# jgrss/cultionet

Hardware: AMD Instinct MI355X
Metric: train_chips_per_sec (higher is better)
Workload: dtype f32

## Files before the change

### cultionet_amd/csrc/cn_wgrad.hip

```cpp
#include <cstdlib>
#include "cn_common.h"
#include "cn_profile.h"
#include "cn_slicesum.h"

#define WG_MAX_TAPS 9
#define WG_BC 32
#define WG_NS 4
#define WG_NB 13
#define WG_KS 8
#define WG_U 4
#define WG_KB 16

struct CnWgradGeom {
  int N;
  int A, Hs, Ws; long sbs; long scs;
  int Bc, Hb, Wb; long bbs; long bcs;
  double flops;
  int s;
  int T;
  int offy[WG_MAX_TAPS], offx[WG_MAX_TAPS];
  int min_oy, min_ox;
  long sa;
  int PR, Wsp, pitch_s;
  int rows_b, pitch_b, plane_b;
  int a_tiles;
  int chunks_per_img, total_chunks, chunks_per_split;
  int b_lds_off;
  int buf_stride;
  int nbuf;
  int colsplit;
  int G, spg;
  const float* gS[4];
  const float* gB[4];
  float* gdW[4];
  long slice_stride;
  int grid_x, grid_y, grid_z;
  int mq_lo, mq_hi;
};

typedef __attribute__((address_space(3))) void* cn_lds_ptr;
typedef const __attribute__((address_space(1))) void* cn_gbl_ptr;

__device__ float cn_zero_line[64];

__device__ __forceinline__ void cn_glds4(const float* src, float* lds_wave_base) {
  __builtin_amdgcn_global_load_lds((cn_gbl_ptr)src, (cn_lds_ptr)lds_wave_base, 4, 0, 0);
}

template <int T>
__global__ __launch_bounds__(256) void cn_wgrad_kernel(const float* __restrict__ S, const float* __restrict__ Bg,
                                                      float* __restrict__ dW, const CnWgradGeom g) {
  extern __shared__ __attribute__((aligned(16))) float smem[];

  const int tid = threadIdx.x, lane = tid & 63, wid = tid >> 6;
  const int half = lane >> 5, l31 = lane & 31;
  const int at = wid % g.a_tiles, kp = wid / g.a_tiles, kparts = 4 / g.a_tiles;
  int bx, by, bz;
  if (!cn_xcd_block(g.grid_x, g.grid_y, g.grid_x * g.grid_y * g.grid_z, bx, by, bz)) return;
  const int a0 = by * g.a_tiles * 32;
  const int b0 = bx * WG_BC;
  const int npix = g.PR * g.Wsp;
  const float* zero = cn_zero_line + lane;

  int so[WG_NS];
#pragma unroll
  for (int i = 0; i < WG_NS; ++i) {
    const int e = lane + i * 64;
    if (e < npix) {
      const int r = e / g.Wsp, c = e - r * g.Wsp;
      so[i] = (r << 16) | ((c < g.Ws) ? c : 0xFFFF);
    } else {
      so[i] = -2;
    }
  }
  int bo[WG_NB];
#pragma unroll
  for (int i = 0; i < WG_NB; ++i) {
    const int e = lane + i * 64;
    if (e < g.plane_b) {
      const int r = e / g.pitch_b;
      bo[i] = (r << 16) | (e - r * g.pitch_b);
    } else {
      bo[i] = -1;
    }
  }

  int boff[T];
#pragma unroll
  for (int j = 0; j < T; ++j) {
    const int n = j * 32 + l31;
    const int bl = n / T, t = n - bl * T;
    boff[j] = bl * g.plane_b + (g.offy[t] - g.min_oy) * g.pitch_b + (g.offx[t] - g.min_ox) + half * g.s;
  }
  const int aoff = (at * 32 + l31) * g.pitch_s + half;

  f32x16 acc[T];
#pragma unroll
  for (int j = 0; j < T; ++j)
#pragma unroll
    for (int r = 0; r < 16; ++r) acc[j][r] = 0.f;

  const int HWs = g.Hs * g.Ws, HWb = g.Hb * g.Wb;
  const int arows = g.a_tiles * 32;
  int chunk = bz * g.chunks_per_split;
  int chunk_end = chunk + g.chunks_per_split;
  if (chunk_end > g.total_chunks) chunk_end = g.total_chunks;

  const int steps = npix >> 1;
  const int q_begin = (steps * kp) / kparts, q_end = (steps * (kp + 1)) / kparts;
  const int e_begin = q_begin * 2;
  const int r_begin = e_begin / g.Wsp, c_begin = e_begin - r_begin * g.Wsp;

  auto stage = [&](int ck, int buf) {
    float* s_lds = smem + buf * g.buf_stride;
    float* b_lds = s_lds + g.b_lds_off;
    const int n = ck / g.chunks_per_img;
    const int gy0 = (ck - n * g.chunks_per_img) * g.PR;
    const int pr = (g.Hs - gy0 < g.PR) ? g.Hs - gy0 : g.PR;
    const float* Sn = S + (long)n * g.sbs + (long)gy0 * g.Ws;
    for (int a = wid; a < arows; a += 4) {
      const bool aok = (a0 + a) < g.A;
      const float* Sa = Sn + (long)(a0 + a) * g.scs;
#pragma unroll
      for (int i = 0; i < WG_NS; ++i) {
        if (i * 64 < npix) {
          if (so[i] != -2) {
            const int r = so[i] >> 16, c = so[i] & 0xFFFF;
            const float* src = (aok && c != 0xFFFF && r < pr) ? Sa + r * g.Ws + c : zero;
            cn_glds4(src, s_lds + a * g.pitch_s + i * 64);
          }
        }
      }
    }
    const float* Bn = Bg + (long)n * g.bbs;
    const int iy0 = gy0 * g.s + g.min_oy;
    for (int bl = wid; bl < WG_BC; bl += 4) {
      const bool bok = (b0 + bl) < g.Bc;
      const float* Bb = Bn + (long)(b0 + bl) * g.bcs;
#pragma unroll
      for (int i = 0; i < WG_NB; ++i) {
        if (i * 64 < g.plane_b) {
          if (bo[i] >= 0) {
            const int iy = iy0 + (bo[i] >> 16), ix = g.min_ox + (bo[i] & 0xFFFF);
            const float* src = (bok && iy >= 0 && iy < g.Hb && ix >= 0 && ix < g.Wb) ? Bb + iy * g.Wb + ix : zero;
            cn_glds4(src, b_lds + bl * g.plane_b + i * 64);
          }
        }
      }
    }
  };

  int cur = 0;
  if (chunk < chunk_end && g.nbuf == 2) stage(chunk, 0);
  for (; chunk < chunk_end; ++chunk) {
    if (g.nbuf == 1) {
      __syncthreads();
      stage(chunk, 0);
    }
    __syncthreads();
    if (g.nbuf == 2 && chunk + 1 < chunk_end) stage(chunk + 1, cur ^ 1);
    const float* s_lds = smem + cur * g.buf_stride;
    const float* b_lds = s_lds + g.b_lds_off;
    int r = r_begin, c = c_begin;
    for (int q = q_begin; q < q_end; ++q) {
      const float av = s_lds[aoff + r * g.Wsp + c];
      const int bbase = (r * g.s) * g.pitch_b + c * g.s;
#pragma unroll
      for (int j = 0; j < T; ++j) {
        const float bv = b_lds[boff[j] + bbase];
        acc[j] = __builtin_amdgcn_mfma_f32_32x32x2f32(av, bv, acc[j], 0, 0, 0);
      }
      c += 2;
      if (c >= g.Wsp) { c = 0; ++r; }
    }
    if (g.nbuf == 2) cur ^= 1;
  }

#pragma unroll
  for (int j = 0; j < T; ++j) {
    const int n = j * 32 + l31;
    const int bl = n / T;
    const bool bok = (b0 + bl) < g.Bc;
#pragma unroll
    for (int r = 0; r < 16; ++r) {
      const int a = a0 + at * 32 + (r & 3) + 8 * (r >> 2) + 4 * half;
      if (bok && a < g.A) atomicAdd(dW + (long)a * g.sa + (long)b0 * T + n, acc[j][r]);
    }
  }
}

__device__ float cn_zero_line16[256];

#ifdef CNW_STAMP
__device__ unsigned long long cnw_stamps[256];
#define CNW_ST() do { if (do_stamp && stamp_i < 256) cnw_stamps[stamp_i++] = __builtin_amdgcn_s_memtime(); } while (0)
extern "C" int cn_wgrad_read_stamps(unsigned long long* out) {
  return hipMemcpyFromSymbol(out, HIP_SYMBOL(cnw_stamps), sizeof(unsigned long long) * 256) == hipSuccess ? 0 : -2;
}
#else
#define CNW_ST() do { } while (0)
#endif

__device__ __forceinline__ void cn_glds16(const float* src, float* lds_wave_base) {
  __builtin_amdgcn_global_load_lds((cn_gbl_ptr)src, (cn_lds_ptr)lds_wave_base, 16, 0, 0);
}

template <int T, int S_>
__global__ __launch_bounds__(256) void cn_wgrad_vec_kernel(const float* __restrict__ S0, const float* __restrict__ Bg0,
                                                          float* __restrict__ dW0, const CnWgradGeom g) {
  extern __shared__ __attribute__((aligned(16))) float smem[];
  const int tid = threadIdx.x, lane = tid & 63;
  const int wid = __builtin_amdgcn_readfirstlane(tid >> 6);
  const int half = lane >> 5, l31 = lane & 31;
  const int at = wid % g.a_tiles, kp = wid / g.a_tiles, kparts = 4 / g.a_tiles;
  int bx, by, bz;
  if (!cn_xcd_block(g.grid_x, g.grid_y, g.grid_x * g.grid_y * g.grid_z, bx, by, bz)) return;
  const int grp = g.G > 1 ? bz / g.spg : 0;
  const int split = bz - grp * g.spg;
  const float* __restrict__ S = g.G > 1 ? g.gS[grp] : S0;
  const float* __restrict__ Bg = g.G > 1 ? g.gB[grp] : Bg0;
  float* __restrict__ dW = (g.G > 1 && g.slice_stride == 0) ? g.gdW[grp] : dW0;
  const int a0 = by * g.a_tiles * 32;
  const int b0 = bx * WG_BC;
  const int npix = g.PR * g.Ws;
  const int n4s = npix >> 2;
  const int n4b = g.plane_b >> 2;
  const float* zero = cn_zero_line16 + 4 * lane;
  const int HWs = g.Hs * g.Ws, HWb = g.Hb * g.Wb;

  int boff[T], ox[T];
#pragma unroll
  for (int j = 0; j < T; ++j) {
    const int n = j * 32 + l31;
    const int bl = n / T, t = n - bl * T;
    boff[j] = bl * g.plane_b + (g.offy[t] - g.min_oy) * g.Wb + (g.offx[t] - g.min_ox) + half * g.s;
    ox[j] = g.offx[t] + half * g.s;
  }
  const int aoff = (at * 32 + l31) * g.pitch_s + half;

  f32x16 acc[T];
#pragma unroll
  for (int j = 0; j < T; ++j)
#pragma unroll
    for (int r = 0; r < 16; ++r) acc[j][r] = 0.f;

  const int arows = g.a_tiles * 32;
  int chunk = split * g.chunks_per_split;
  int chunk_end = chunk + g.chunks_per_split;
  if (chunk_end > g.total_chunks) chunk_end = g.total_chunks;

  const int steps = npix >> 1;
  const int q_begin = (steps * kp) / kparts, q_end = (steps * (kp + 1)) / kparts;
  const int e_begin = q_begin * 2;
  const int r_begin = e_begin / g.Ws, c_begin = e_begin - r_begin * g.Ws;

  constexpr unsigned WG_IDLE = 0xFFFFFFFFu;
  unsigned so[WG_KS], bo[WG_KB];
  {
    const int nsp = arows * n4s, nbp = WG_BC * n4b;
#pragma unroll
    for (int k = 0; k < WG_KS; ++k) {
      const int p = (wid + 4 * k) * 64 + lane;
      const int a = p / n4s, pc = p - a * n4s;
      so[k] = (p < nsp && (a0 + a) < g.A) ? (unsigned)(((long)(a0 + a) * g.scs + 4 * pc) * 4) : WG_IDLE;
    }
#pragma unroll
    for (int k = 0; k < WG_KB; ++k) {
      const int p = (wid + 4 * k) * 64 + lane;
      const int bl = p / n4b, pi = p - bl * n4b;
      bo[k] = (p < nbp && (b0 + bl) < g.Bc) ? (unsigned)(((long)(b0 + bl) * g.bcs + 4 * pi) * 4) : WG_IDLE;
    }
  }
  auto stage = [&](int ck, int buf) {
    float* s_lds = smem + buf * g.buf_stride;
    float* b_lds = s_lds + g.b_lds_off;
    const int n = ck / g.chunks_per_img;
    const int gy0 = (ck - n * g.chunks_per_img) * g.PR;
    const int nsp = arows * n4s, nbp = WG_BC * n4b;
    {
      const int fs0 = gy0 * g.Ws;
      const char* sbase = reinterpret_cast<const char*>(S + (long)n * g.sbs + fs0);
      if (fs0 + npix <= (int)g.scs) {
#pragma unroll
        for (int k = 0; k < WG_KS; ++k)
          if ((wid + 4 * k) * 64 < nsp && so[k] != WG_IDLE)
            cn_glds16(reinterpret_cast<const float*>(sbase + so[k]), s_lds + (wid + 4 * k) * 256);
      } else {
#pragma unroll
        for (int k = 0; k < WG_KS; ++k) {
          if ((wid + 4 * k) * 64 < nsp && so[k] != WG_IDLE) {
            const int p = (wid + 4 * k) * 64 + lane;
            const int pc = p % n4s;
            const bool ok = (fs0 + 4 * pc + 3) < (int)g.scs;
            const float* src = ok ? reinterpret_cast<const float*>(sbase + so[k]) : zero;
            cn_glds16(src, s_lds + (wid + 4 * k) * 256);
          }
        }
      }
    }
    {
      const int start = (gy0 * g.s + g.min_oy) * g.Wb + g.min_ox;
      const int f0 = (start >> 2) << 2;
      const char* bbase = reinterpret_cast<const char*>(Bg + (long)n * g.bbs + f0);
      if (f0 >= 0 && f0 + g.plane_b <= (int)g.bcs) {
#pragma unroll
        for (int k = 0; k < WG_KB; ++k)
          if ((wid + 4 * k) * 64 < nbp && bo[k] != WG_IDLE)
            cn_glds16(reinterpret_cast<const float*>(bbase + bo[k]), b_lds + (wid + 4 * k) * 256);
      } else {
#pragma unroll
        for (int k = 0; k < WG_KB; ++k) {
          if ((wid + 4 * k) * 64 < nbp && bo[k] != WG_IDLE) {
            const int p = (wid + 4 * k) * 64 + lane;
            const int fq = f0 + 4 * (p % n4b);
            const bool ok = fq >= 0 && (fq + 3) < (int)g.bcs;
            const float* src = ok ? reinterpret_cast<const float*>(bbase + bo[k]) : zero;
            cn_glds16(src, b_lds + (wid + 4 * k) * 256);
          }
        }
      }
    }
  };

  int cur = 0;
#ifdef CNW_STAMP
  const bool do_stamp = T == 9 && S_ == 1 && blockIdx.x == 8 && tid == 0;
  int stamp_i = 0;
#endif
  CNW_ST();
  if (chunk < chunk_end && g.nbuf == 2) stage(chunk, 0);
  for (; chunk < chunk_end; ++chunk) {
    CNW_ST();
    if (g.nbuf == 1) {
      __syncthreads();
      stage(chunk, 0);
    }
    __syncthreads();
    CNW_ST();
    if (g.nbuf == 2 && chunk + 1 < chunk_end) stage(chunk + 1, cur ^ 1);
    CNW_ST();
    const float* s_lds = smem + cur * g.buf_stride;
    const float* b_lds = s_lds + g.b_lds_off;
    const int gy0c = (chunk % g.chunks_per_img) * g.PR;
    const int start = (gy0c * g.s + g.min_oy) * g.Wb + g.min_ox;
    const int sh = start - ((start >> 2) << 2);
    {
      const int nq_row = g.Ws >> 1;
      const int q_lo = (nq_row * kp) / kparts, q_hi = (nq_row * (kp + 1)) / kparts;
      const int seg0 = min(max(g.mq_lo, q_lo), q_hi), seg1 = max(min(g.mq_hi, q_hi), seg0);
      for (int r = 0; r < g.PR; ++r) {
        const float* ap = s_lds + aoff + r * g.Ws;
        const float* bp[T];
#pragma unroll
        for (int j = 0; j < T; ++j) bp[j] = b_lds + boff[j] + sh + (r * S_) * g.Wb;
        int q = q_lo;
        for (; q < seg0; ++q) {
          const float av = ap[2 * q];
          const int cs = 2 * q * S_;
          float bv[T];
#pragma unroll
          for (int j = 0; j < T; ++j) bv[j] = bp[j][cs];
#pragma unroll
          for (int j = 0; j < T; ++j) {
            const float b_ = ((unsigned)(cs + ox[j]) < (unsigned)g.Wb) ? bv[j] : 0.f;
            acc[j] = __builtin_amdgcn_mfma_f32_32x32x2f32(av, b_, acc[j], 0, 0, 0);
          }
        }
        CNW_ST();
        if constexpr (T == 1) {
          for (; q + WG_U <= seg1; q += WG_U) {
            const float* apq = ap + 2 * q;
#pragma unroll
            for (int u = 0; u < WG_U; ++u)
              acc[0] = __builtin_amdgcn_mfma_f32_32x32x2f32(apq[2 * u], (bp[0] + 2 * q * S_)[2 * u * S_], acc[0], 0, 0, 0);
          }
        } else {
          constexpr int GS = 2;
          const int ng = (seg1 - q) / GS;
          if (ng > 0) {
            float a0[GS], a1[GS], b0[GS][T], b1[GS][T];
#define WG_LOADG(qq_, a_, b_)                                                    \
  {                                                                              \
    const float* apq_ = ap + 2 * (qq_);                                          \
    _Pragma("unroll") for (int u = 0; u < GS; ++u) a_[u] = apq_[2 * u];          \
    _Pragma("unroll") for (int j = 0; j < T; ++j) {                              \
      const float* bq_ = bp[j] + 2 * (qq_) * S_;                                 \
      _Pragma("unroll") for (int u = 0; u < GS; ++u) b_[u][j] = bq_[2 * u * S_]; \
    }                                                                            \
  }
#define WG_MFMAG(a_, b_)                                                                                   \
  {                                                                                                        \
    _Pragma("unroll") for (int u = 0; u < GS; ++u)                                                         \
        _Pragma("unroll") for (int j = 0; j < T; ++j)                                                      \
            acc[j] = __builtin_amdgcn_mfma_f32_32x32x2f32(a_[u], b_[u][j], acc[j], 0, 0, 0);               \
  }
            WG_LOADG(q, a0, b0);
            int i = 0;
            for (; i + 2 <= ng; i += 2) {
              WG_LOADG(q + GS * (i + 1), a1, b1);
              WG_MFMAG(a0, b0);
              if (i + 2 < ng) WG_LOADG(q + GS * (i + 2), a0, b0);
              WG_MFMAG(a1, b1);
            }
            if (i < ng) WG_MFMAG(a0, b0);
#undef WG_LOADG
#undef WG_MFMAG
            q += GS * ng;
          }
        }
        CNW_ST();
        for (; q < seg1; ++q) {
          const float av = ap[2 * q];
          float bv[T];
#pragma unroll
          for (int j = 0; j < T; ++j) bv[j] = bp[j][2 * q * S_];
#pragma unroll
          for (int j = 0; j < T; ++j) acc[j] = __builtin_amdgcn_mfma_f32_32x32x2f32(av, bv[j], acc[j], 0, 0, 0);
        }
        for (; q < q_hi; ++q) {
          const float av = ap[2 * q];
          const int cs = 2 * q * S_;
          float bv[T];
#pragma unroll
          for (int j = 0; j < T; ++j) bv[j] = bp[j][cs];
#pragma unroll
          for (int j = 0; j < T; ++j) {
            const float b_ = ((unsigned)(cs + ox[j]) < (unsigned)g.Wb) ? bv[j] : 0.f;
            acc[j] = __builtin_amdgcn_mfma_f32_32x32x2f32(av, b_, acc[j], 0, 0, 0);
          }
        }
      }
    }
    CNW_ST();
    if (g.nbuf == 2) cur ^= 1;
  }
  CNW_ST();

  if (kparts > 1) {
    __syncthreads();
    float* red = smem;
    if (kp > 0) {
      float* rp = red + (long)((kp - 1) * g.a_tiles + at) * (T * 16 * 64) + lane;
#pragma unroll
      for (int j = 0; j < T; ++j)
#pragma unroll
        for (int r = 0; r < 16; ++r) rp[(j * 16 + r) * 64] = acc[j][r];
    }
    __syncthreads();
    if (kp > 0) return;
    for (int k = 1; k < kparts; ++k) {
      const float* rp = red + (long)((k - 1) * g.a_tiles + at) * (T * 16 * 64) + lane;
#pragma unroll
      for (int j = 0; j < T; ++j)
#pragma unroll
        for (int r = 0; r < 16; ++r) acc[j][r] += rp[(j * 16 + r) * 64];
    }
  }
  float* dWs = dW + (long)bz * g.slice_stride;
#pragma unroll
  for (int j = 0; j < T; ++j) {
    const int n = j * 32 + l31;
    const int bl = n / T;
    const bool bok = (b0 + bl) < g.Bc;
#pragma unroll
    for (int r = 0; r < 16; ++r) {
      const int a = a0 + at * 32 + (r & 3) + 8 * (r >> 2) + 4 * half;
      if (bok && a < g.A) {
        if (g.slice_stride != 0) dWs[(long)a * g.sa + (long)b0 * T + n] = acc[j][r];
        else atomicAdd(dW + (long)a * g.sa + (long)b0 * T + n, acc[j][r]);
      }
    }
  }
}

#define WG3_WAVES 12
#define WG3_KS 3
#define WG3_KB 6
template <int S_>
__global__ __launch_bounds__(WG3_WAVES * 64) void cn_wgrad_vec3_kernel(const float* __restrict__ S0,
                                                                       const float* __restrict__ Bg0,
                                                                       float* __restrict__ dW0, const CnWgradGeom g) {
  extern __shared__ __attribute__((aligned(16))) float smem[];
  constexpr int T = 3;
  const int tid = threadIdx.x, lane = tid & 63;
  const int wid = __builtin_amdgcn_readfirstlane(tid >> 6);
  const int half = lane >> 5, l31 = lane & 31;
  const int at = wid % g.a_tiles;
  const int ky = (wid / g.a_tiles) % 3;
  const int kp = wid / (g.a_tiles * 3), kparts = WG3_WAVES / (g.a_tiles * 3);
  int bx, by, bz;
  if (!cn_xcd_block(g.grid_x, g.grid_y, g.grid_x * g.grid_y * g.grid_z, bx, by, bz)) return;
  const int grp = g.G > 1 ? bz / g.spg : 0;
  const int split = bz - grp * g.spg;
  const float* __restrict__ S = g.G > 1 ? g.gS[grp] : S0;
  const float* __restrict__ Bg = g.G > 1 ? g.gB[grp] : Bg0;
  float* __restrict__ dW = (g.G > 1 && g.slice_stride == 0) ? g.gdW[grp] : dW0;
  const int a0 = by * g.a_tiles * 32;
  const int b0 = bx * WG_BC;
  const int npix = g.PR * g.Ws;
  const int n4s = npix >> 2;
  const int n4b = g.plane_b >> 2;
  const float* zero = cn_zero_line16 + 4 * lane;

  int boff[T], ox[T];
#pragma unroll
  for (int j = 0; j < T; ++j) {
    const int n = j * 32 + l31;
    const int bl = n / 3, t = ky * 3 + (n - bl * 3);
    boff[j] = bl * g.plane_b + (g.offy[t] - g.min_oy) * g.Wb + (g.offx[t] - g.min_ox) + half * g.s;
    ox[j] = g.offx[t] + half * g.s;
  }
  const int aoff = (at * 32 + l31) * g.pitch_s + half;

  f32x16 acc[T];
#pragma unroll
  for (int j = 0; j < T; ++j)
#pragma unroll
    for (int r = 0; r < 16; ++r) acc[j][r] = 0.f;

  const int arows = g.a_tiles * 32;
  int chunk = split * g.chunks_per_split;
  int chunk_end = chunk + g.chunks_per_split;
  if (chunk_end > g.total_chunks) chunk_end = g.total_chunks;

  constexpr unsigned WG_IDLE = 0xFFFFFFFFu;
  unsigned so[WG3_KS], bo[WG3_KB];
  {
    const int nsp = arows * n4s, nbp = WG_BC * n4b;
#pragma unroll
    for (int k = 0; k < WG3_KS; ++k) {
      const int p = (wid + WG3_WAVES * k) * 64 + lane;
      const int a = p / n4s, pc = p - a * n4s;
      so[k] = (p < nsp && (a0 + a) < g.A) ? (unsigned)(((long)(a0 + a) * g.scs + 4 * pc) * 4) : WG_IDLE;
    }
#pragma unroll
    for (int k = 0; k < WG3_KB; ++k) {
      const int p = (wid + WG3_WAVES * k) * 64 + lane;
      const int bl = p / n4b, pi = p - bl * n4b;
      bo[k] = (p < nbp && (b0 + bl) < g.Bc) ? (unsigned)(((long)(b0 + bl) * g.bcs + 4 * pi) * 4) : WG_IDLE;
    }
  }
  auto stage = [&](int ck, int buf) {
    float* s_lds = smem + buf * g.buf_stride;
    float* b_lds = s_lds + g.b_lds_off;
    const int n = ck / g.chunks_per_img;
    const int gy0 = (ck - n * g.chunks_per_img) * g.PR;
    const int nsp = arows * n4s, nbp = WG_BC * n4b;
    {
      const int fs0 = gy0 * g.Ws;
      const char* sbase = reinterpret_cast<const char*>(S + (long)n * g.sbs + fs0);
      const bool inside = fs0 + npix <= (int)g.scs;
#pragma unroll
      for (int k = 0; k < WG3_KS; ++k) {
        if ((wid + WG3_WAVES * k) * 64 < nsp && so[k] != WG_IDLE) {
          const float* src = reinterpret_cast<const float*>(sbase + so[k]);
          if (!inside) {
            const int p = (wid + WG3_WAVES * k) * 64 + lane;
            if (!((fs0 + 4 * (p % n4s) + 3) < (int)g.scs)) src = zero;
          }
          cn_glds16(src, s_lds + (wid + WG3_WAVES * k) * 256);
        }
      }
    }
    {
      const int start = (gy0 * g.s + g.min_oy) * g.Wb + g.min_ox;
      const int f0 = (start >> 2) << 2;
      const char* bbase = reinterpret_cast<const char*>(Bg + (long)n * g.bbs + f0);
      const bool inside = f0 >= 0 && f0 + g.plane_b <= (int)g.bcs;
#pragma unroll
      for (int k = 0; k < WG3_KB; ++k) {
        if ((wid + WG3_WAVES * k) * 64 < nbp && bo[k] != WG_IDLE) {
          const float* src = reinterpret_cast<const float*>(bbase + bo[k]);
          if (!inside) {
            const int p = (wid + WG3_WAVES * k) * 64 + lane;
            const int fq = f0 + 4 * (p % n4b);
            if (!(fq >= 0 && (fq + 3) < (int)g.bcs)) src = zero;
          }
          cn_glds16(src, b_lds + (wid + WG3_WAVES * k) * 256);
        }
      }
    }
  };

  int cur = 0;
  if (chunk < chunk_end && g.nbuf == 2) stage(chunk, 0);
  for (; chunk < chunk_end; ++chunk) {
    if (g.nbuf == 1) {
      __syncthreads();
      stage(chunk, 0);
    }
    __syncthreads();
    if (g.nbuf == 2 && chunk + 1 < chunk_end) stage(chunk + 1, cur ^ 1);
    const float* s_lds = smem + cur * g.buf_stride;
    const float* b_lds = s_lds + g.b_lds_off;
    const int gy0c = (chunk % g.chunks_per_img) * g.PR;
    const int start = (gy0c * g.s + g.min_oy) * g.Wb + g.min_ox;
    const int sh = start - ((start >> 2) << 2);
    const int nq_row = g.Ws >> 1;
    const int q_lo = (nq_row * kp) / kparts, q_hi = (nq_row * (kp + 1)) / kparts;
    const int seg0 = min(max(g.mq_lo, q_lo), q_hi), seg1 = max(min(g.mq_hi, q_hi), seg0);
    for (int r = 0; r < g.PR; ++r) {
      const float* ap = s_lds + aoff + r * g.Ws;
      const float* bp[T];
#pragma unroll
      for (int j = 0; j < T; ++j) bp[j] = b_lds + boff[j] + sh + (r * S_) * g.Wb;
      int q = q_lo;
      for (; q < seg0; ++q) {
        const float av = ap[2 * q];
        const int cs = 2 * q * S_;
        float bv[T];
#pragma unroll
        for (int j = 0; j < T; ++j) bv[j] = bp[j][cs];
#pragma unroll
        for (int j = 0; j < T; ++j) {
          const float b_ = ((unsigned)(cs + ox[j]) < (unsigned)g.Wb) ? bv[j] : 0.f;
          acc[j] = __builtin_amdgcn_mfma_f32_32x32x2f32(av, b_, acc[j], 0, 0, 0);
        }
      }
      {
        constexpr int GS = 3;
        const int ng = (seg1 - q) / GS;
        if (ng > 0) {
          float a0[GS], a1[GS], b0[GS][T], b1[GS][T];
#define WG3_LOADG(qq_, a_, b_)                                                   \
  {                                                                              \
    const float* apq_ = ap + 2 * (qq_);                                          \
    _Pragma("unroll") for (int u = 0; u < GS; ++u) a_[u] = apq_[2 * u];          \
    _Pragma("unroll") for (int j = 0; j < T; ++j) {                              \
      const float* bq_ = bp[j] + 2 * (qq_) * S_;                                 \
      _Pragma("unroll") for (int u = 0; u < GS; ++u) b_[u][j] = bq_[2 * u * S_]; \
    }                                                                            \
  }
#define WG3_MFMAG(a_, b_)                                                                                  \
  {                                                                                                        \
    _Pragma("unroll") for (int u = 0; u < GS; ++u)                                                         \
        _Pragma("unroll") for (int j = 0; j < T; ++j)                                                      \
            acc[j] = __builtin_amdgcn_mfma_f32_32x32x2f32(a_[u], b_[u][j], acc[j], 0, 0, 0);               \
  }
          WG3_LOADG(q, a0, b0);
          int i = 0;
          for (; i + 2 <= ng; i += 2) {
            WG3_LOADG(q + GS * (i + 1), a1, b1);
            WG3_MFMAG(a0, b0);
            if (i + 2 < ng) WG3_LOADG(q + GS * (i + 2), a0, b0);
            WG3_MFMAG(a1, b1);
          }
          if (i < ng) WG3_MFMAG(a0, b0);
#undef WG3_LOADG
#undef WG3_MFMAG
          q += GS * ng;
        }
      }
      for (; q < seg1; ++q) {
        const float av = ap[2 * q];
        float bv[T];
#pragma unroll
        for (int j = 0; j < T; ++j) bv[j] = bp[j][2 * q * S_];
#pragma unroll
        for (int j = 0; j < T; ++j) acc[j] = __builtin_amdgcn_mfma_f32_32x32x2f32(av, bv[j], acc[j], 0, 0, 0);
      }
      for (; q < q_hi; ++q) {
        const float av = ap[2 * q];
        const int cs = 2 * q * S_;
        float bv[T];
#pragma unroll
        for (int j = 0; j < T; ++j) bv[j] = bp[j][cs];
#pragma unroll
        for (int j = 0; j < T; ++j) {
          const float b_ = ((unsigned)(cs + ox[j]) < (unsigned)g.Wb) ? bv[j] : 0.f;
          acc[j] = __builtin_amdgcn_mfma_f32_32x32x2f32(av, b_, acc[j], 0, 0, 0);
        }
      }
    }
    if (g.nbuf == 2) cur ^= 1;
  }

  if (kparts > 1) {
    __syncthreads();
    float* red = smem;
    const int slot = ky * g.a_tiles + at;
    if (kp > 0) {
      float* rp = red + (long)((kp - 1) * g.a_tiles * 3 + slot) * (T * 16 * 64) + lane;
#pragma unroll
      for (int j = 0; j < T; ++j)
#pragma unroll
        for (int r = 0; r < 16; ++r) rp[(j * 16 + r) * 64] = acc[j][r];
    }
    __syncthreads();
    if (kp > 0) return;
    for (int k = 1; k < kparts; ++k) {
      const float* rp = red + (long)((k - 1) * g.a_tiles * 3 + slot) * (T * 16 * 64) + lane;
#pragma unroll
      for (int j = 0; j < T; ++j)
#pragma unroll
        for (int r = 0; r < 16; ++r) acc[j][r] += rp[(j * 16 + r) * 64];
    }
  }
  float* dWs = dW + (long)bz * g.slice_stride;
#pragma unroll
  for (int j = 0; j < T; ++j) {
    const int n = j * 32 + l31;
    const int bl = n / 3, t = ky * 3 + (n - bl * 3);
    const bool bok = (b0 + bl) < g.Bc;
#pragma unroll
    for (int r = 0; r < 16; ++r) {
      const int a = a0 + at * 32 + (r & 3) + 8 * (r >> 2) + 4 * half;
      if (bok && a < g.A) {
        float* d = (g.slice_stride != 0 ? dWs : dW) + (long)a * g.sa + (long)(b0 + bl) * 9 + t;
        if (g.slice_stride != 0) *d = acc[j][r];
        else atomicAdd(d, acc[j][r]);
      }
    }
  }
}

struct CnWgradReduceArgs {
  const float* part; long slice_stride; int nslices; long n;
  float* dW[4];
};
__global__ __launch_bounds__(256) void cn_wgrad_reduce_kernel(const CnWgradReduceArgs a) {
  const long i = blockIdx.x * 256L + threadIdx.x;
  if (i >= a.n) return;
  const float* part = a.part + (long)blockIdx.z * a.nslices * a.slice_stride;
  float* dW = a.dW[blockIdx.z];
  float s0 = 0.f, s1 = 0.f;
  int k = blockIdx.y;
  for (; k + (int)gridDim.y < a.nslices; k += 2 * gridDim.y) {
    s0 += part[(long)k * a.slice_stride + i];
    s1 += part[(long)(k + gridDim.y) * a.slice_stride + i];
  }
  if (k < a.nslices) s0 += part[(long)k * a.slice_stride + i];
  if (gridDim.y == 1) dW[i] += s0 + s1;
  else atomicAdd(dW + i, s0 + s1);
}

template <int T>
static int cn_wgrad_launch_vec(const float* S, const float* Bg, float* dW, CnWgradGeom g, float* ws, long ws_floats,
                               hipStream_t stream) {
  if (g.scs % 4 || g.bcs % 4 || g.sbs % 4 || g.bbs % 4 || (g.Ws & 1)) return CN_ERR_ARG;
  g.Wsp = g.Ws;
  g.PR = 128 / g.Ws;
  if (g.PR < 1) g.PR = 1;
  if (g.PR > g.Hs) g.PR = g.Hs;
  while (g.PR > 1 && (g.PR * g.Ws) % 4 != 0) --g.PR;
  if ((g.PR * g.Ws) % 4 != 0 && g.Ws % 2 == 0 && 2 * g.Ws <= 256) g.PR = 2;
  if ((g.PR * g.Ws) % 4 != 0 || g.PR * g.Ws > 256) return CN_ERR_ARG;
  int max_oy = g.min_oy, max_ox = g.min_ox;
  for (int t = 0; t < g.T; ++t) {
    if (g.offy[t] > max_oy) max_oy = g.offy[t];
    if (g.offx[t] > max_ox) max_ox = g.offx[t];
  }
  g.rows_b = (g.PR - 1) * g.s + (max_oy - g.min_oy) + 1;
  g.pitch_b = g.Wb;
  g.plane_b = ((g.rows_b - 1) * g.Wb + (g.Ws - 1) * g.s + (max_ox - g.min_ox) + 4 + 3) / 4 * 4;
  if (WG_BC * g.plane_b > WG_KB * 4 * 256) return CN_ERR_ARG;
  g.pitch_s = g.PR * g.Ws;
  g.a_tiles = g.A > 32 ? 2 : 1;
  size_t lds;
  for (;;) {
    g.b_lds_off = (g.a_tiles * 32 * g.pitch_s + 255) / 256 * 256;
    g.buf_stride = g.b_lds_off + (WG_BC * g.plane_b + 255) / 256 * 256;
    lds = (size_t)g.buf_stride * sizeof(float);
    if ((lds <= 160 * 1024 && g.a_tiles * 32 * g.pitch_s <= WG_KS * 4 * 256) || g.a_tiles == 1) break;
    g.a_tiles >>= 1;
  }
  if (lds > 160 * 1024 || g.a_tiles * 32 * g.pitch_s > WG_KS * 4 * 256) return CN_ERR_ARG;
  g.nbuf = (2 * lds <= 160 * 1024) ? 2 : 1;
  lds *= g.nbuf;
  {
    const size_t red = (size_t)(4 / g.a_tiles - 1) * g.a_tiles * T * 16 * 64 * sizeof(float);
    if (red > lds) lds = red;
  }
  g.chunks_per_img = (g.Hs + g.PR - 1) / g.PR;
  g.total_chunks = g.N * g.chunks_per_img;
  const int gx = (g.Bc + WG_BC - 1) / WG_BC, gy = (g.A + g.a_tiles * 32 - 1) / (g.a_tiles * 32);
  if (g.G < 1) {
    g.G = 1;
    g.gS[0] = S; g.gB[0] = Bg; g.gdW[0] = dW;
  }
  for (int i = 0; i < g.G; ++i)
    if ((reinterpret_cast<uintptr_t>(g.gS[i]) & 15) || (reinterpret_cast<uintptr_t>(g.gB[i]) & 15)) return CN_ERR_ARG;
  const int slots = (lds * 2 <= 160 * 1024) ? 512 : 256;
  int splits = slots / (gx * gy * g.G);
  if (splits > g.total_chunks) splits = g.total_chunks;
  if (splits < 1) splits = 1;
  g.chunks_per_split = (g.total_chunks + splits - 1) / splits;
  splits = (g.total_chunks + g.chunks_per_split - 1) / g.chunks_per_split;
  static bool attr_set = false;
  if (!attr_set) {
    (void)hipFuncSetAttribute((const void*)cn_wgrad_vec_kernel<T, 1>, hipFuncAttributeMaxDynamicSharedMemorySize,
                              160 * 1024);
    (void)hipFuncSetAttribute((const void*)cn_wgrad_vec_kernel<T, 2>, hipFuncAttributeMaxDynamicSharedMemorySize,
                              160 * 1024);
    attr_set = true;
  }
  if (g.s != 1 && g.s != 2) return CN_ERR_ARG;
  {
    const int nq_row = g.Ws / 2;
    int lo = (-g.min_ox + 2 * g.s - 1) / (2 * g.s);
    if (lo < 0) lo = 0;
    int hi_num = g.Wb - max_ox - g.s;
    int hi = hi_num <= 0 ? 0 : (hi_num + 2 * g.s - 1) / (2 * g.s);
    if (lo > nq_row) lo = nq_row;
    if (hi > nq_row) hi = nq_row;
    if (hi < lo) hi = lo;
    g.mq_lo = lo;
    g.mq_hi = hi;
  }
  cn_prof_name("cn_wgrad_vec_kernel<%d, %d>", T, g.s == 1 ? 1 : 2);
  cn_prof_desc("wgrad_vec<%d> G%d N%d A%d %dx%d Bc%d %dx%d s%d grid%dx%dx%d nbuf%d", T, g.G, g.N, g.A, g.Hs, g.Ws, g.Bc,
               g.Hb, g.Wb, g.s, gx, gy, splits, g.nbuf);
  g.spg = splits;
  g.grid_x = gx; g.grid_y = gy; g.grid_z = splits * g.G;
  const dim3 grid(cn_xcd_grid((long)gx * gy * splits * g.G));
  const int kparts = 4 / g.a_tiles;
  const long dw_floats = (long)g.A * g.sa;
  const long nslices = splits;
  float* out = g.gdW[0];
  g.slice_stride = 0;
  if (nslices >= 16 && ws != nullptr && nslices * g.G * dw_floats <= ws_floats) {
    g.slice_stride = dw_floats;
    out = ws;
  }
  if (T == 9) cn_prof_name("cn_wgrad_vec3_kernel<%d>", g.s == 1 ? 1 : 2);
  cn_prof_bytes(4.0 * g.G * ((double)g.N * g.A * g.Hs * g.Ws + (double)g.N * g.Bc * g.Hb * g.Wb + (double)dw_floats));
  cn_prof_before(stream);
  if (T == 9) {
    static bool attr3 = false;
    if (!attr3) {
      (void)hipFuncSetAttribute((const void*)cn_wgrad_vec3_kernel<1>, hipFuncAttributeMaxDynamicSharedMemorySize, 160 * 1024);
      (void)hipFuncSetAttribute((const void*)cn_wgrad_vec3_kernel<2>, hipFuncAttributeMaxDynamicSharedMemorySize, 160 * 1024);
      attr3 = true;
    }
    if (g.s == 1)
      CN_LAUNCH((cn_wgrad_vec3_kernel<1>), grid, dim3(WG3_WAVES * 64), lds, stream, g.gS[0], g.gB[0], out, g);
    else
      CN_LAUNCH((cn_wgrad_vec3_kernel<2>), grid, dim3(WG3_WAVES * 64), lds, stream, g.gS[0], g.gB[0], out, g);
  } else if (g.s == 1)
    CN_LAUNCH((cn_wgrad_vec_kernel<T, 1>), grid, dim3(256), lds, stream, g.gS[0], g.gB[0], out, g);
  else
    CN_LAUNCH((cn_wgrad_vec_kernel<T, 2>), grid, dim3(256), lds, stream, g.gS[0], g.gB[0], out, g);
  cn_prof_after(stream, T == 9 ? 2 : 3, g.flops * g.G);
  if (g.slice_stride != 0) {
    CnSliceSum js[4] = {};
    for (int i = 0; i < g.G; ++i) {
      js[i].part = ws + (long)i * nslices * g.slice_stride; js[i].dw = g.gdW[i]; js[i].slice_stride = g.slice_stride;
      js[i].n = dw_floats; js[i].nslices = (int)nslices; js[i].kind = 0;
    }
    if (cn_ss_push(js, g.G)) return cn_check_launch();
    CnWgradReduceArgs ra = {ws, g.slice_stride, (int)nslices, dw_floats, {g.gdW[0], g.gdW[1], g.gdW[2], g.gdW[3]}};
    CN_LAUNCH(cn_wgrad_reduce_kernel,
                       dim3((unsigned)((dw_floats + 255) / 256), nslices > 128 ? 16 : 1, g.G), dim3(256), 0, stream,
                       ra);
  }
  return cn_check_launch();
}

template <int T>
static int cn_wgrad_launch_t(const float* S, const float* Bg, float* dW, CnWgradGeom g, hipStream_t stream) {
  g.Wsp = (g.Ws + 1) & ~1;
  if (g.Wsp > 64 * WG_NS) return CN_ERR_LDS;
  g.PR = 128 / g.Wsp;
  if (g.PR < 1) g.PR = 1;
  if (g.PR > g.Hs) g.PR = g.Hs;
  int max_oy = g.min_oy, max_ox = g.min_ox;
  for (int t = 0; t < g.T; ++t) {
    if (g.offy[t] > max_oy) max_oy = g.offy[t];
    if (g.offx[t] > max_ox) max_ox = g.offx[t];
  }
  for (;;) {
    g.rows_b = (g.PR - 1) * g.s + (max_oy - g.min_oy) + 1;
    g.pitch_b = (g.Wsp - 1) * g.s + (max_ox - g.min_ox) + 1;
    g.plane_b = g.rows_b * g.pitch_b;
    if (g.plane_b <= 64 * WG_NB || g.PR == 1) break;
    --g.PR;
  }
  if (g.plane_b > 64 * WG_NB) return CN_ERR_LDS;
  g.pitch_s = (g.PR * g.Wsp) | 1;
  g.a_tiles = g.A > 64 ? 4 : (g.A > 32 ? 2 : 1);
  if (g.a_tiles == 4) g.a_tiles = 2;
  size_t lds;
  for (;;) {
    g.b_lds_off = (g.a_tiles * 32 * g.pitch_s + 3) / 4 * 4;
    g.buf_stride = (g.b_lds_off + WG_BC * g.plane_b + 3) / 4 * 4;
    lds = (size_t)g.buf_stride * sizeof(float);
    if (lds <= 160 * 1024 || g.a_tiles == 1) break;
    g.a_tiles >>= 1;
  }
  if (lds > 160 * 1024) return CN_ERR_LDS;
  g.nbuf = (2 * lds <= 160 * 1024) ? 2 : 1;
  lds *= g.nbuf;
  g.chunks_per_img = (g.Hs + g.PR - 1) / g.PR;
  g.total_chunks = g.N * g.chunks_per_img;
  const int gx = (g.Bc + WG_BC - 1) / WG_BC, gy = (g.A + g.a_tiles * 32 - 1) / (g.a_tiles * 32);
  int splits = (768 + gx * gy - 1) / (gx * gy);
  if (splits > g.total_chunks) splits = g.total_chunks;
  if (splits < 1) splits = 1;
  g.chunks_per_split = (g.total_chunks + splits - 1) / splits;
  splits = (g.total_chunks + g.chunks_per_split - 1) / g.chunks_per_split;
  static bool attr_set = false;
  if (!attr_set) {
    (void)hipFuncSetAttribute((const void*)cn_wgrad_kernel<T>, hipFuncAttributeMaxDynamicSharedMemorySize,
                              160 * 1024);
    attr_set = true;
  }
  cn_prof_name("cn_wgrad_kernel<%d>", T);
  cn_prof_desc("wgrad_dw<%d> N%d A%d %dx%d Bc%d %dx%d s%d grid%dx%dx%d", T, g.N, g.A, g.Hs, g.Ws, g.Bc, g.Hb, g.Wb, g.s,
               gx, gy, splits);
  g.grid_x = gx; g.grid_y = gy; g.grid_z = splits;
  cn_prof_before(stream);
  CN_LAUNCH((cn_wgrad_kernel<T>), dim3(cn_xcd_grid((long)gx * gy * splits)), dim3(256), lds, stream, S, Bg,
                     dW, g);
  cn_prof_after(stream, T == 9 ? 2 : 3, g.flops);
  return cn_check_launch();
}

struct CnPadSet {
  const float* src; long sbs; long scs;
  float* dst; int C, H, W, Wp, cs;
};
#define CN_PAD_MAX_SETS 8
struct CnPadArgs {
  CnPadSet set[CN_PAD_MAX_SETS];
  int cbegin[CN_PAD_MAX_SETS + 1];
  int nsets;
};

__global__ __launch_bounds__(256) void cn_pad_planes_kernel(const CnPadArgs a) {
  int si = 0;
#pragma unroll 1
  for (int i = 1; i < a.nsets; ++i)
    if ((int)blockIdx.y >= a.cbegin[i]) si = i;
  const CnPadSet& p = a.set[si];
  const int c = blockIdx.y - a.cbegin[si], b = blockIdx.z;
  const float* sp = p.src + b * p.sbs + (long)c * p.scs;
  float* dp = p.dst + ((long)b * p.C + c) * p.cs;
  for (int i = blockIdx.x * 256 + threadIdx.x; i < p.cs; i += gridDim.x * 256) {
    const int r = i / p.Wp, col = i - r * p.Wp;
    dp[i] = (r < p.H && col < p.W) ? sp[r * p.W + col] : 0.f;
  }
}

static int cn_pad_planes(CnPadArgs& a, int B, hipStream_t stream) {
  if (a.nsets == 0) return CN_OK;
  int cs = 0, ctot = 0;
  for (int i = 0; i < a.nsets; ++i) {
    a.cbegin[i] = ctot;
    ctot += a.set[i].C;
    if (a.set[i].cs > cs) cs = a.set[i].cs;
  }
  a.cbegin[a.nsets] = ctot;
  int bx = (cs + 1023) / 1024;
  if (bx < 1) bx = 1;
  CN_LAUNCH(cn_pad_planes_kernel, dim3(bx, ctot, B), dim3(256), 0, stream, a);
  return cn_check_launch();
}

static int cn_wgrad_generic_g(int G, const float* const* Ss, long sbs, int A, int Hs, int Ws, const float* const* Bgs,
                              long bbs, int Bc, int Hb, int Wb, int s, int KH, int KW, int dil, int pad,
                              float* const* dWs, int N, float* ws, long ws_floats, hipStream_t stream) {
  if (G < 1 || G > 4) return CN_ERR_ARG;
  CnWgradGeom g = {};
  g.N = N; g.A = A; g.Hs = Hs; g.Ws = Ws; g.sbs = sbs; g.Bc = Bc; g.Hb = Hb; g.Wb = Wb; g.bbs = bbs; g.s = s;
  g.scs = (long)Hs * Ws; g.bcs = (long)Hb * Wb;
  g.T = KH * KW;
  if (N <= 0 || A <= 0 || Bc <= 0 || Hs <= 0 || Ws <= 0) return CN_OK;
  g.flops = 2.0 * N * Hs * Ws * (double)A * Bc * g.T;
  for (int ky = 0; ky < KH; ++ky)
    for (int kx = 0; kx < KW; ++kx) {
      g.offy[ky * KW + kx] = ky * dil - pad;
      g.offx[ky * KW + kx] = kx * dil - pad;
    }
  g.min_oy = -pad; g.min_ox = -pad;
  g.sa = (long)Bc * g.T;
  if (g.T != 1 && g.T != 9) return CN_ERR_ARG;
  g.G = G;
  for (int i = 0; i < G; ++i) { g.gS[i] = Ss[i]; g.gB[i] = Bgs[i]; g.gdW[i] = dWs[i]; }
  const bool ws_ok = ws != nullptr && (reinterpret_cast<uintptr_t>(ws) & 15) == 0;
  int rc = g.T == 1 ? cn_wgrad_launch_vec<1>(Ss[0], Bgs[0], dWs[0], g, ws_ok ? ws : nullptr, ws_floats, stream)
                    : cn_wgrad_launch_vec<9>(Ss[0], Bgs[0], dWs[0], g, ws_ok ? ws : nullptr, ws_floats, stream);
  if (rc != CN_ERR_ARG) return rc;
  if (ws_ok) {
    const int Wsp = (Ws + 1) & ~1;
    const long scs = ((long)Hs * Wsp + 3) / 4 * 4, bcs = ((long)Hb * Wb + 3) / 4 * 4;
    const long need_s = (long)N * A * scs, need_b = (long)N * Bc * bcs;
    CnWgradGeom gp = g;
    CnPadArgs pa = {};
    float* w = ws;
    long need = 0;
    bool any_s = false, any_b = false;
    for (int i = 0; i < G; ++i) {
      const bool s_ok = (g.scs % 4 == 0) && (sbs % 4 == 0) && !(Ws & 1) && !(reinterpret_cast<uintptr_t>(Ss[i]) & 15);
      const bool b_ok = (g.bcs % 4 == 0) && (bbs % 4 == 0) && !(reinterpret_cast<uintptr_t>(Bgs[i]) & 15);
      any_s |= !s_ok;
      any_b |= !b_ok;
    }
    for (int i = 0; i < G && any_s; ++i) {
      pa.set[pa.nsets++] = {Ss[i], sbs, (long)Hs * Ws, w, A, Hs, Ws, Wsp, (int)scs};
      gp.gS[i] = w; w += need_s; need += need_s;
    }
    for (int i = 0; i < G && any_b; ++i) {
      int same = -1;
      for (int j = 0; j < i; ++j)
        if (Bgs[j] == Bgs[i]) same = j;
      if (same >= 0) { gp.gB[i] = gp.gB[same]; continue; }
      pa.set[pa.nsets++] = {Bgs[i], bbs, (long)Hb * Wb, w, Bc, Hb, Wb, Wb, (int)bcs};
      gp.gB[i] = w; w += need_b; need += need_b;
    }
    if (any_s) { gp.Ws = Wsp; gp.scs = scs; gp.sbs = (long)A * scs; }
    if (any_b) { gp.bcs = bcs; gp.bbs = (long)Bc * bcs; }
    if (need <= ws_floats) {
      const int r = cn_pad_planes(pa, N, stream);
      if (r != CN_OK) return r;
      float* wrest = ws + (need + 3) / 4 * 4;
      const long nrest = ws_floats - (need + 3) / 4 * 4;
      rc = g.T == 1 ? cn_wgrad_launch_vec<1>(gp.gS[0], gp.gB[0], dWs[0], gp, wrest, nrest, stream)
                    : cn_wgrad_launch_vec<9>(gp.gS[0], gp.gB[0], dWs[0], gp, wrest, nrest, stream);
      if (rc != CN_ERR_ARG) return rc;
    }
  }
  for (int i = 0; i < G; ++i) {
    CnWgradGeom g1 = g;
    g1.G = 0;
    rc = g.T == 1 ? cn_wgrad_launch_t<1>(Ss[i], Bgs[i], dWs[i], g1, stream)
                  : cn_wgrad_launch_t<9>(Ss[i], Bgs[i], dWs[i], g1, stream);
    if (rc != CN_OK) return rc;
  }
  return CN_OK;
}

static int cn_wgrad_generic(const float* S, long sbs, int A, int Hs, int Ws, const float* Bg, long bbs, int Bc,
                            int Hb, int Wb, int s, int KH, int KW, int dil, int pad, float* dW, int N, float* ws,
                            long ws_floats, hipStream_t stream) {
  return cn_wgrad_generic_g(1, &S, sbs, A, Hs, Ws, &Bg, bbs, Bc, Hb, Wb, s, KH, KW, dil, pad, &dW, N, ws, ws_floats,
                            stream);
}

extern "C" int cn_conv2d_bwd_weight_grouped_f32(int G, const float* const* xs, long xbs, const float* const* dys,
                                                long dybs, float* const* dws, int B, int Cin, int Hin, int Win,
                                                int Cout, int KH, int KW, int stride, int pad, int dil, float* ws,
                                                long ws_floats, void* stream) {
  if (stride < 1) return CN_ERR_ARG;
  const int Hout = (Hin + 2 * pad - dil * (KH - 1) - 1) / stride + 1;
  const int Wout = (Win + 2 * pad - dil * (KW - 1) - 1) / stride + 1;
  return cn_wgrad_generic_g(G, dys, dybs, Cout, Hout, Wout, xs, xbs, Cin, Hin, Win, stride, KH, KW, dil, pad, dws, B,
                            ws, ws_floats, (hipStream_t)stream);
}

extern "C" int cn_conv2d_bwd_weight_f32(const float* x, long xbs, const float* dy, long dybs, float* dw, int B,
                                        int Cin, int Hin, int Win, int Cout, int KH, int KW, int stride, int pad,
                                        int dil, float* ws, long ws_floats, void* stream) {
  if (stride < 1) return CN_ERR_ARG;
  const int Hout = (Hin + 2 * pad - dil * (KH - 1) - 1) / stride + 1;
  const int Wout = (Win + 2 * pad - dil * (KW - 1) - 1) / stride + 1;
  return cn_wgrad_generic(dy, dybs, Cout, Hout, Wout, x, xbs, Cin, Hin, Win, stride, KH, KW, dil, pad, dw, B, ws,
                          ws_floats, (hipStream_t)stream);
}

extern "C" int cn_conv_transpose2d_bwd_weight_f32(const float* x, long xbs, const float* dy, long dybs, float* dw,
                                                  int B, int Cin, int Hin, int Win, int Cout, int KH, int KW,
                                                  int stride, int pad, int out_pad, float* ws, long ws_floats,
                                                  void* stream) {
  if (out_pad < 0 || (out_pad > 0 && out_pad >= stride)) return CN_ERR_ARG;
  const int Hout = (Hin - 1) * stride - 2 * pad + KH + out_pad;
  const int Wout = (Win - 1) * stride - 2 * pad + KW + out_pad;
  return cn_wgrad_generic(x, xbs, Cin, Hin, Win, dy, dybs, Cout, Hout, Wout, stride, KH, KW, 1, pad, dw, B, ws,
                          ws_floats, (hipStream_t)stream);
}
```

Measured before the change: 382.1.

## Add specialized small-spatial 3x3 weight-gradient kernel with split-K reduction

Adds a new MFMA weight-gradient kernel for 3x3 convolutions with small spatial extents. It uses 12 waves per block, splits the pixel reduction across waves and sums the parts in LDS, and chooses the tiling with a cost model. Per-slice partial results are then summed by the existing slice-sum/reduce path. The goal is to raise occupancy and parallelism on small feature maps where the generic vector kernel leaves the GPU underused. The cost is a large amount of extra code plus extra workspace traffic for the partial slices.

```diff
diff --git a/cultionet_amd/csrc/cn_wgrad.hip b/cultionet_amd/csrc/cn_wgrad.hip
--- a/cultionet_amd/csrc/cn_wgrad.hip
+++ b/cultionet_amd/csrc/cn_wgrad.hip
@@ -714,6 +714,192 @@
   }
 }
 
+#define WS3_WAVES 12
+#define WS3_THREADS (WS3_WAVES * 64)
+#define WS3_NS 10
+#define WS3_NB 16
+#define WS3_GS 4
+template <int S_>
+__global__ __launch_bounds__(WS3_THREADS) void cn_wgrad_small3_kernel(const CnWgradGeom g, float* __restrict__ part) {
+  extern __shared__ __attribute__((aligned(16))) float smem[];
+  constexpr int T = 3;
+  const int tid = threadIdx.x, lane = tid & 63;
+  const int wid = __builtin_amdgcn_readfirstlane(tid >> 6);
+  const int half = lane >> 5, l31 = lane & 31;
+  const int at = wid % g.a_tiles;
+  const int ky = (wid / g.a_tiles) % 3;
+  const int kp = wid / (g.a_tiles * 3), kparts = WS3_WAVES / (g.a_tiles * 3);
+  int bx, by, bz;
+  if (!cn_xcd_block(g.grid_x, g.grid_y, g.grid_x * g.grid_y * g.grid_z, bx, by, bz)) return;
+  const int grp = bz / g.spg;
+  const int split = bz - grp * g.spg;
+  const float* __restrict__ S = g.gS[grp];
+  const float* __restrict__ Bg = g.gB[grp];
+  const int a0 = by * g.a_tiles * 32;
+  const int b0 = bx * WG_BC;
+  const int npix = g.PR;
+  const int arows = g.a_tiles * 32;
+  const int nrb = g.rows_b * g.Wb;
+  const int front = g.pitch_b;
+  const int HWs = g.Hs * g.Ws, HWb = g.Hb * g.Wb;
+
+  int boff[T], ox[T];
+#pragma unroll
+  for (int j = 0; j < T; ++j) {
+    const int n = j * 32 + l31;
+    const int bl = n / 3, t = ky * 3 + (n - bl * 3);
+    boff[j] = bl * g.plane_b + front + (g.offy[t] - g.min_oy) * g.Wb + g.offx[t];
+    ox[j] = g.offx[t];
+  }
+  const int aoff = (at * 32 + l31) * g.pitch_s + half;
+
+  f32x16 acc[T];
+#pragma unroll
+  for (int j = 0; j < T; ++j)
+#pragma unroll
+    for (int r = 0; r < 16; ++r) acc[j][r] = 0.f;
+
+  int chunk = split * g.chunks_per_split;
+  int chunk_end = chunk + g.chunks_per_split;
+  if (chunk_end > g.total_chunks) chunk_end = g.total_chunks;
+
+  const int ns = arows * npix, nb = WG_BC * nrb;
+  const int s_da = WS3_THREADS / npix, s_di = WS3_THREADS - s_da * npix;
+  const int b_dl = WS3_THREADS / nrb, b_dk = WS3_THREADS - b_dl * nrb;
+  const int s_a0 = tid / npix, s_i0 = tid - s_a0 * npix;
+  const int b_l0 = tid / nrb, b_k0 = tid - b_l0 * nrb;
+  float sv[WS3_NS], bv[WS3_NB];
+  auto load = [&](int ck) {
+    const int n = ck / g.chunks_per_img;
+    const int p0 = (ck - n * g.chunks_per_img) * npix;
+    const int f0 = (p0 / g.Ws * S_ + g.min_oy) * g.Wb;
+    const float* Sn = S + (long)n * g.sbs + p0;
+    const float* Bn = Bg + (long)n * g.bbs + f0;
+    int a = s_a0, i = s_i0, bl = b_l0, kk = b_k0;
+    asm volatile("" : "+v"(a), "+v"(i), "+v"(bl), "+v"(kk));
+#pragma unroll
+    for (int k = 0; k < WS3_NS; ++k) {
+      const bool ok = tid + WS3_THREADS * k < ns && a0 + a < g.A && p0 + i < HWs;
+      sv[k] = ok ? Sn[(long)(a0 + a) * g.scs + i] : 0.f;
+      a += s_da; i += s_di;
+      if (i >= npix) { i -= npix; ++a; }
+    }
+#pragma unroll
+    for (int k = 0; k < WS3_NB; ++k) {
+      const bool ok = tid + WS3_THREADS * k < nb && b0 + bl < g.Bc && (unsigned)(f0 + kk) < (unsigned)HWb;
+      bv[k] = ok ? Bn[(long)(b0 + bl) * g.bcs + kk] : 0.f;
+      bl += b_dl; kk += b_dk;
+      if (kk >= nrb) { kk -= nrb; ++bl; }
+    }
+  };
+  auto store = [&](int buf) {
+    float* s_lds = smem + buf * g.buf_stride;
+    float* b_lds = s_lds + g.b_lds_off;
+    int a = s_a0, i = s_i0, bl = b_l0, kk = b_k0;
+    asm volatile("" : "+v"(a), "+v"(i), "+v"(bl), "+v"(kk));
+#pragma unroll
+    for (int k = 0; k < WS3_NS; ++k) {
+      if (tid + WS3_THREADS * k < ns) s_lds[a * g.pitch_s + i] = sv[k];
+      a += s_da; i += s_di;
+      if (i >= npix) { i -= npix; ++a; }
+    }
+#pragma unroll
+    for (int k = 0; k < WS3_NB; ++k) {
+      if (tid + WS3_THREADS * k < nb) b_lds[bl * g.plane_b + front + kk] = bv[k];
+      bl += b_dl; kk += b_dk;
+      if (kk >= nrb) { kk -= nrb; ++bl; }
+    }
+  };
+
+  const int steps = npix >> 1;
+  const int q_begin = (steps * kp) / kparts, q_end = (steps * (kp + 1)) / kparts;
+  int cur = 0;
+  if (tid == 0) smem[2 * g.buf_stride] = 0.f;
+  if (chunk < chunk_end) {
+    load(chunk);
+    store(0);
+  }
+  for (; chunk < chunk_end; ++chunk) {
+    __syncthreads();
+    const bool more = chunk + 1 < chunk_end;
+    if (more) load(chunk + 1);
+    const float* s_lds = smem + cur * g.buf_stride;
+    const float* b_lds = s_lds + g.b_lds_off;
+    const int n = chunk / g.chunks_per_img;
+    const int p0 = (chunk - n * g.chunks_per_img) * npix;
+    const int yf = p0 / g.Ws;
+    int x, base;
+    {
+      const int p = p0 - yf * g.Ws + 2 * q_begin + half;
+      const int ry = p / g.Ws;
+      x = p - ry * g.Ws;
+      base = S_ * (ry * g.Wb + x);
+    }
+    const int wrap = S_ * (g.Wb - g.Ws);
+    const int zslot = 2 * g.buf_stride - (s_lds + g.b_lds_off - smem);
+    const float* ap = s_lds + aoff;
+    for (int q = q_begin; q < q_end; q += WS3_GS) {
+      int bi[WS3_GS][T];
+#pragma unroll
+      for (int u = 0; u < WS3_GS; ++u) {
+#pragma unroll
+        for (int j = 0; j < T; ++j) bi[u][j] = ((unsigned)(S_ * x + ox[j]) < (unsigned)g.Wb) ? boff[j] + base : zslot;
+        x += 2;
+        base += 2 * S_;
+        if (x >= g.Ws) { x -= g.Ws; base += wrap; }
+      }
+      float av[WS3_GS], bw[WS3_GS][T];
+#pragma unroll
+      for (int u = 0; u < WS3_GS; ++u) {
+        av[u] = ap[2 * (q + u)];
+#pragma unroll
+        for (int j = 0; j < T; ++j) bw[u][j] = b_lds[bi[u][j]];
+      }
+      __builtin_amdgcn_sched_barrier(0);
+#pragma unroll
+      for (int u = 0; u < WS3_GS; ++u)
+#pragma unroll
+        for (int j = 0; j < T; ++j) acc[j] = __builtin_amdgcn_mfma_f32_32x32x2f32(av[u], bw[u][j], acc[j], 0, 0, 0);
+    }
+    if (more) store(cur ^ 1);
+    cur ^= 1;
+  }
+
+  if (kparts > 1) {
+    __syncthreads();
+    float* red = smem;
+    const int slot = ky * g.a_tiles + at;
+    if (kp > 0) {
+      float* rp = red + (long)((kp - 1) * g.a_tiles * 3 + slot) * (T * 16 * 64) + lane;
+#pragma unroll
+      for (int j = 0; j < T; ++j)
+#pragma unroll
+        for (int r = 0; r < 16; ++r) rp[(j * 16 + r) * 64] = acc[j][r];
+    }
+    __syncthreads();
+    if (kp > 0) return;
+    for (int k = 1; k < kparts; ++k) {
+      const float* rp = red + (long)((k - 1) * g.a_tiles * 3 + slot) * (T * 16 * 64) + lane;
+#pragma unroll
+      for (int j = 0; j < T; ++j)
+#pragma unroll
+        for (int r = 0; r < 16; ++r) acc[j][r] += rp[(j * 16 + r) * 64];
+    }
+  }
+  float* dWs = part + (long)bz * g.slice_stride;
+#pragma unroll
+  for (int j = 0; j < T; ++j) {
+    const int n = j * 32 + l31;
+    const int bl = n / 3, t = ky * 3 + (n - bl * 3);
+    const bool bok = (b0 + bl) < g.Bc;
+#pragma unroll
+    for (int r = 0; r < 16; ++r) {
+      const int a = a0 + at * 32 + (r & 3) + 8 * (r >> 2) + 4 * half;
+      if (bok && a < g.A) dWs[(long)a * g.sa + (long)(b0 + bl) * 9 + t] = acc[j][r];
+    }
+  }
+}
+
 struct CnWgradReduceArgs {
   const float* part; long slice_stride; int nslices; long n;
   float* dW[4];
@@ -853,6 +1039,112 @@
                        dim3((unsigned)((dw_floats + 255) / 256), nslices > 128 ? 16 : 1, g.G), dim3(256), 0, stream,
                        ra);
   }
+  return cn_check_launch();
+}
+
+static int cn_wgrad_launch_small3(CnWgradGeom g, float* ws, long ws_floats, hipStream_t stream) {
+  if (g.T != 9 || ws == nullptr || (g.s != 1 && g.s != 2)) return CN_ERR_ARG;
+  if (g.Ws < 2 || (long)g.Hs * g.Ws > 2500 || g.Wb > 64) return CN_ERR_ARG;
+  const long hws = (long)g.Hs * g.Ws;
+  if (!(g.s == 1 && hws <= 625 && g.Bc <= 128) && !(g.s == 2 && hws <= 169 && g.Bc >= 256)) return CN_ERR_ARG;
+  int max_oy = g.min_oy, max_ox = g.min_ox;
+  for (int t = 0; t < 9; ++t) {
+    if (g.offy[t] > max_oy) max_oy = g.offy[t];
+    if (g.offx[t] > max_ox) max_ox = g.offx[t];
+  }
+  const int front = g.min_ox < 0 ? -g.min_ox : 0;
+  const int HWs = g.Hs * g.Ws;
+  const long dw_floats = (long)g.A * g.sa;
+  const int gx = (g.Bc + WG_BC - 1) / WG_BC;
+  double best = 0.0;
+  CnWgradGeom pick = g;
+  bool found = false;
+  for (int at = 1; at <= 4; at *= 2) {
+    const int kparts = 4 / at, arows = 32 * at;
+    const int gran = 2 * kparts * WS3_GS;
+    const int gy = (g.A + arows - 1) / arows;
+    for (int cpi = 1; cpi <= 64; ++cpi) {
+      const int npix = ((HWs + cpi - 1) / cpi + gran - 1) / gran * gran;
+      if (npix > 256) continue;
+      if ((npix - gran) * cpi >= HWs && cpi > 1) continue;
+      const int ry_max = (g.Ws - 1 + npix - 1) / g.Ws;
+      const int rows_b = ry_max * g.s + (max_oy - g.min_oy) + 1;
+      const int nrb = rows_b * g.Wb;
+      if (arows * npix > WS3_THREADS * WS3_NS || WG_BC * nrb > WS3_THREADS * WS3_NB) continue;
+      int plane_b = front + (rows_b - 1) * g.Wb + g.s * (g.Ws - 1) + max_ox + 1;
+      if (plane_b < front + nrb) plane_b = front + nrb;
+      plane_b |= 1;
+      const int pitch_s = npix + 1;
+      const int b_lds_off = (arows * pitch_s + 3) / 4 * 4;
+      const int buf_stride = (b_lds_off + WG_BC * plane_b + 3) / 4 * 4;
+      if ((2L * buf_stride + 4) * 4 > 160 * 1024) continue;
+      const int total = g.N * cpi, base = gx * gy * g.G;
+      int splits = 256 / base;
+      if (splits < 1) splits = 1;
+      if (splits > total) splits = total;
+      const int cps = (total + splits - 1) / splits;
+      splits = (total + cps - 1) / cps;
+      if ((long)splits * g.G * dw_floats > ws_floats) continue;
+      const long blocks = (long)base * splits;
+      const int rounds = (int)((blocks + 255) / 256);
+      const double chunk_cyc = 8.0 * at * 9 * npix + 1500.0;
+      const double cost = rounds * (cps * chunk_cyc + 4000.0) + 8.0 * splits * g.G * dw_floats / 2000.0;
+      if (found && cost >= best) continue;
+      found = true;
+      best = cost;
+      pick = g;
+      pick.a_tiles = at;
+      pick.PR = npix;
+      pick.rows_b = rows_b;
+      pick.pitch_b = front;
+      pick.plane_b = plane_b;
+      pick.pitch_s = pitch_s;
+      pick.b_lds_off = b_lds_off;
+      pick.buf_stride = buf_stride;
+      pick.chunks_per_img = cpi;
+      pick.total_chunks = total;
+      pick.chunks_per_split = cps;
+      pick.spg = splits;
+      pick.grid_x = gx; pick.grid_y = gy; pick.grid_z = splits * g.G;
+    }
+  }
+  if (!found) return CN_ERR_ARG;
+  g = pick;
+  g.nbuf = 2;
+  g.slice_stride = dw_floats;
+  size_t lds = ((size_t)2 * g.buf_stride + 4) * sizeof(float);
+  {
+    const size_t red = (size_t)(4 / g.a_tiles - 1) * g.a_tiles * 3 * 3 * 16 * 64 * sizeof(float);
+    if (red > lds) lds = red;
+  }
+  if (lds > 160 * 1024) return CN_ERR_ARG;
+  static bool attr = false;
+  if (!attr) {
+    (void)hipFuncSetAttribute((const void*)cn_wgrad_small3_kernel<1>, hipFuncAttributeMaxDynamicSharedMemorySize, 160 * 1024);
+    (void)hipFuncSetAttribute((const void*)cn_wgrad_small3_kernel<2>, hipFuncAttributeMaxDynamicSharedMemorySize, 160 * 1024);
+    attr = true;
+  }
+  const long nslices = g.spg;
+  cn_prof_name("cn_wgrad_small3_kernel<%d>", g.s);
+  cn_prof_desc("wgrad_small3 G%d N%d A%d %dx%d Bc%d %dx%d s%d at%d px%d grid%dx%dx%d", g.G, g.N, g.A, g.Hs, g.Ws, g.Bc,
+               g.Hb, g.Wb, g.s, g.a_tiles, g.PR, g.grid_x, g.grid_y, g.spg);
+  cn_prof_bytes(4.0 * g.G * ((double)g.N * g.A * g.Hs * g.Ws + (double)g.N * g.Bc * g.Hb * g.Wb + (double)dw_floats));
+  cn_prof_before(stream);
+  const dim3 grid(cn_xcd_grid((long)g.grid_x * g.grid_y * g.grid_z));
+  if (g.s == 1)
+    CN_LAUNCH((cn_wgrad_small3_kernel<1>), grid, dim3(WS3_THREADS), lds, stream, g, ws);
+  else
+    CN_LAUNCH((cn_wgrad_small3_kernel<2>), grid, dim3(WS3_THREADS), lds, stream, g, ws);
+  cn_prof_after(stream, 2, g.flops * g.G);
+  CnSliceSum js[4] = {};
+  for (int i = 0; i < g.G; ++i) {
+    js[i].part = ws + (long)i * nslices * g.slice_stride; js[i].dw = g.gdW[i]; js[i].slice_stride = g.slice_stride;
+    js[i].n = dw_floats; js[i].nslices = (int)nslices; js[i].kind = 0;
+  }
+  if (cn_ss_push(js, g.G)) return cn_check_launch();
+  CnWgradReduceArgs ra = {ws, g.slice_stride, (int)nslices, dw_floats, {g.gdW[0], g.gdW[1], g.gdW[2], g.gdW[3]}};
+  CN_LAUNCH(cn_wgrad_reduce_kernel, dim3((unsigned)((dw_floats + 255) / 256), nslices > 128 ? 16 : 1, g.G), dim3(256),
+            0, stream, ra);
   return cn_check_launch();
 }
 
@@ -977,6 +1269,10 @@
   g.G = G;
   for (int i = 0; i < G; ++i) { g.gS[i] = Ss[i]; g.gB[i] = Bgs[i]; g.gdW[i] = dWs[i]; }
   const bool ws_ok = ws != nullptr && (reinterpret_cast<uintptr_t>(ws) & 15) == 0;
+  if (g.T == 9 && ws_ok) {
+    const int rc3 = cn_wgrad_launch_small3(g, ws, ws_floats, stream);
+    if (rc3 != CN_ERR_ARG) return rc3;
+  }
   int rc = g.T == 1 ? cn_wgrad_launch_vec<1>(Ss[0], Bgs[0], dWs[0], g, ws_ok ? ws : nullptr, ws_floats, stream)
                     : cn_wgrad_launch_vec<9>(Ss[0], Bgs[0], dWs[0], g, ws_ok ? ws : nullptr, ws_floats, stream);
   if (rc != CN_ERR_ARG) return rc;
```

Result: faster. 388.3 (median of 6 runs) (+1.6%).
